# LioQing/wgpu-3dgs-core

Hardware: AMD Instinct MI355X
Metric: Msplats/s @1080p (Gaussians per second through proj+sort+blend; 3 frames in flight on 3 priority streams) (higher is better)
Workload: dtype f32; 1 GPU; 1M synthetic Gaussians, SH degree 0 (ShNone/RotScale 48 B), 1920x1080; gaussians=1000000, visible=708615, pairs=2550276, launches_per_frame=14, parallelism=single GPU, 3 frames in flight on 3 priority streams, frames_in_flight=3, renderer_scratch_copies=3

## Files before the change

### __graft_entry__.py

```python
import os
import sys

ROOT = os.path.dirname(os.path.abspath(__file__))
for p in (ROOT, os.path.join(ROOT, "tools")):
    if p not in sys.path:
        sys.path.insert(0, p)


def build_cpp_mirror_test():
    import subprocess
    out = os.path.join(ROOT, "build")
    os.makedirs(out, exist_ok=True)
    exe = os.path.join(out, "test_mirror")
    subprocess.run(["g++", "-std=c++17", "-O1", "-Wall", "-I" + os.path.join(ROOT, "include"),
                    os.path.join(ROOT, "tests", "cpp", "test_mirror.cpp"), "-o", exe,
                    "-L" + os.path.join(ROOT, "wgpu-3dgs-core_amd", "lib"), "-lgs3d_hip",
                    "-Wl,-rpath,$ORIGIN/../wgpu-3dgs-core_amd/lib"], check=True)
    return exe


def build_cpp_selection_test():
    import subprocess
    out = os.path.join(ROOT, "build")
    os.makedirs(out, exist_ok=True)
    exe = os.path.join(out, "test_selection")
    subprocess.run(["g++", "-std=c++17", "-O1", "-Wall", "-I" + os.path.join(ROOT, "include"),
                    os.path.join(ROOT, "tests", "cpp", "test_selection.cpp"), "-o", exe,
                    "-L" + os.path.join(ROOT, "wgpu-3dgs-core_amd", "lib"), "-lgs3d_hip",
                    "-Wl,-rpath,$ORIGIN/../wgpu-3dgs-core_amd/lib"], check=True)
    return exe


def build_cpp_edit_test():
    import subprocess
    out = os.path.join(ROOT, "build")
    os.makedirs(out, exist_ok=True)
    exe = os.path.join(out, "test_edit")
    subprocess.run(["g++", "-std=c++17", "-O1", "-Wall", "-I" + os.path.join(ROOT, "include"),
                    os.path.join(ROOT, "tests", "cpp", "test_edit.cpp"), "-o", exe,
                    "-L" + os.path.join(ROOT, "wgpu-3dgs-core_amd", "lib"), "-lgs3d_hip",
                    "-Wl,-rpath,$ORIGIN/../wgpu-3dgs-core_amd/lib"], check=True)
    return exe


def build_cpp_history_test():
    import subprocess
    out = os.path.join(ROOT, "build")
    os.makedirs(out, exist_ok=True)
    exe = os.path.join(out, "test_history")
    subprocess.run(["g++", "-std=c++17", "-O1", "-Wall", "-I" + os.path.join(ROOT, "include"),
                    os.path.join(ROOT, "tests", "cpp", "test_history.cpp"), "-o", exe,
                    "-L" + os.path.join(ROOT, "wgpu-3dgs-core_amd", "lib"), "-lgs3d_hip",
                    "-Wl,-rpath,$ORIGIN/../wgpu-3dgs-core_amd/lib"], check=True)
    return exe


def build_cpp_stats_test():
    import subprocess
    out = os.path.join(ROOT, "build")
    os.makedirs(out, exist_ok=True)
    exe = os.path.join(out, "test_stats")
    subprocess.run(["g++", "-std=c++17", "-O1", "-Wall", "-I" + os.path.join(ROOT, "include"),
                    os.path.join(ROOT, "tests", "cpp", "test_stats.cpp"), "-o", exe,
                    "-L" + os.path.join(ROOT, "wgpu-3dgs-core_amd", "lib"), "-lgs3d_hip",
                    "-Wl,-rpath,$ORIGIN/../wgpu-3dgs-core_amd/lib"], check=True)
    return exe


def build_cpp_convert_test():
    import subprocess
    out = os.path.join(ROOT, "build")
    os.makedirs(out, exist_ok=True)
    exe = os.path.join(out, "test_convert")
    subprocess.run(["g++", "-std=c++17", "-O1", "-Wall", "-I" + os.path.join(ROOT, "include"),
                    os.path.join(ROOT, "tests", "cpp", "test_convert.cpp"), "-o", exe,
                    "-L" + os.path.join(ROOT, "wgpu-3dgs-core_amd", "lib"), "-lgs3d_hip",
                    "-Wl,-rpath,$ORIGIN/../wgpu-3dgs-core_amd/lib"], check=True)
    return exe


def build_cpp_contrib_test():
    import subprocess
    out = os.path.join(ROOT, "build")
    os.makedirs(out, exist_ok=True)
    exe = os.path.join(out, "test_contrib")
    subprocess.run(["g++", "-std=c++17", "-O1", "-Wall", "-I" + os.path.join(ROOT, "include"),
                    os.path.join(ROOT, "tests", "cpp", "test_contrib.cpp"), "-o", exe,
                    "-L" + os.path.join(ROOT, "wgpu-3dgs-core_amd", "lib"), "-lgs3d_hip",
                    "-Wl,-rpath,$ORIGIN/../wgpu-3dgs-core_amd/lib"], check=True)
    return exe


def build_cpp_metrics_test():
    import subprocess
    out = os.path.join(ROOT, "build")
    os.makedirs(out, exist_ok=True)
    exe = os.path.join(out, "test_metrics")
    subprocess.run(["g++", "-std=c++17", "-O1", "-Wall", "-I" + os.path.join(ROOT, "include"),
                    os.path.join(ROOT, "tests", "cpp", "test_metrics.cpp"), "-o", exe,
                    "-L" + os.path.join(ROOT, "wgpu-3dgs-core_amd", "lib"), "-lgs3d_hip",
                    "-Wl,-rpath,$ORIGIN/../wgpu-3dgs-core_amd/lib"], check=True)
    return exe


def build_cpp_logf_test():
    import subprocess
    out = os.path.join(ROOT, "build")
    os.makedirs(out, exist_ok=True)
    exe = os.path.join(out, "test_logf")
    subprocess.run(["g++", "-std=c++17", "-O2", "-Wall", "-ffp-contract=off", "-pthread",
                    os.path.join(ROOT, "tests", "cpp", "test_logf.cpp"), "-o", exe], check=True)
    return exe


def build_cpp_fullsize_test():
    import subprocess
    out = os.path.join(ROOT, "build")
    os.makedirs(out, exist_ok=True)
    exe, obj = os.path.join(out, "test_fullsize"), os.path.join(out, "gs_synth.o")
    subprocess.run(["gcc", "-O2", "-std=c11", "-fopenmp", "-c", os.path.join(ROOT, "tools", "gs_synth.c"), "-o", obj], check=True)
    subprocess.run(["g++", "-std=c++17", "-O2", "-Wall", "-I" + os.path.join(ROOT, "include"),
                    os.path.join(ROOT, "tests", "cpp", "test_fullsize.cpp"), obj, "-o", exe, "-fopenmp", "-lm",
                    "-L" + os.path.join(ROOT, "wgpu-3dgs-core_amd", "lib"), "-lgs3d_hip",
                    "-Wl,-rpath,$ORIGIN/../wgpu-3dgs-core_amd/lib"], check=True)
    return exe


def build():
    import importlib.util
    spec = importlib.util.spec_from_file_location(
        "_gs_build", os.path.join(ROOT, "wgpu-3dgs-core_amd", "build.py"))
    b = importlib.util.module_from_spec(spec)
    spec.loader.exec_module(b)
    path = b.build(force=True, verbose=True)
    assert os.path.exists(path)
    from oracle import binding as ob
    ob.build(force=True)
    import synth
    synth.build(force=True)
    build_cpp_mirror_test()
    build_cpp_selection_test()
    build_cpp_edit_test()
    build_cpp_history_test()
    build_cpp_stats_test()
    build_cpp_convert_test()
    build_cpp_contrib_test()
    build_cpp_metrics_test()
    build_cpp_logf_test()
    build_cpp_fullsize_test()
    import wgpu_3dgs_core_amd as gs
    assert gs._capi.load().gs_abi_version() == 1
    print("built:", path)


def smoke():
    import numpy as np
    import synth
    import wgpu_3dgs_core_amd as gs
    from oracle import binding as ob

    dev = gs.Device(0)
    lim = dev.limits()
    print("device:", lim.arch_name.decode(), "CUs", lim.compute_units)
    stream = dev.create_stream()
    pod = gs.GaussianPodWithShSingleCov3dRotScaleConfigs
    g = synth.scene(20000)
    pods = pod.from_gaussian(g)
    W, H = 640, 360
    cam = gs.camera_look_at((0, 0, 0), (0, 0, -1), (0, 1, 0), float(np.deg2rad(60.0)), W, H)
    gt, mt = gs.gaussian_transform_pod(sh_deg=3), gs.model_transform_pod()
    buf = gs.GaussiansBuffer.new_with_pods(dev, pod, pods)
    img = gs.Buffer(dev, size=W * H * 16)
    r = gs.Renderer(dev)
    r.render(stream, buf, gt, mt, cam, img.device_ptr())
    rgba = img.download(stream, np.float32).reshape(H, W, 4)
    st = r.stats()

    ocam = ob.Camera()
    for name, _ in cam._fields_:
        v = getattr(cam, name)
        if hasattr(v, "__len__"):
            getattr(ocam, name)[:] = list(v)
        else:
            setattr(ocam, name, v)
    if os.environ.get("GS3D_RECT_V1") != "1":
        ob.set_rect_version(4 if r.sort_info().tile_masks else 3)
    order = buf.download_order(stream)
    assert np.array_equal(order, ob.spatial_order(pod.sh, pod.cov, pods))
    ref, d, vis, _ = ob.render(pod.sh, pod.cov, pods, ob.gaussian_transform(sh_deg=3),
                               ob.model_transform(), ocam, order=order)
    err = float(np.abs(rgba - ref).max())
    print("smoke: N=%d visible=%d pairs=%d  oracle pairs=%d  RGBA Linf=%g" % (len(g), st.visible, st.pairs, d, err))
    assert st.pairs == d and st.visible == vis
    assert err <= 1e-4, err
    m = gs.image_compare(dev, stream, img.device_ptr(), img.device_ptr(), W, H, ssim=True)
    assert m.identical and m.finite == W * H and m.differing == 0 and m.ssim == 1.0, m
    print("smoke OK")


if __name__ == "__main__":
    build()
    if "--smoke" in sys.argv:
        smoke()
```

### wgpu-3dgs-core_amd/csrc/gs_render_kernels.h

```cpp
#pragma once

#include <type_traits>

#include "gs_device_common.h"

namespace gs {

constexpr int PP_THREADS = 256;
constexpr int PP_ITEMS = 4;
constexpr int PP_CHUNK = PP_THREADS * PP_ITEMS;

struct FrameConsts {
    float M[16];
    float V[16];
    float ISR[9];
    float WS[9];
    float cam_pos[3];
    float fx, fy, cx, cy;
    float near_plane, far_plane;
    float size2, limx, limy, max_std_dev;
    float bg[3];
    uint32_t sh_deg, no_sh0;
    uint32_t width, height;
    uint32_t tiles_x, tiles_y;
    uint32_t band_ty0, band_ty1;
    uint32_t mask_culled_records;
    uint32_t nt_loads;
    uint32_t clip_rect;
    float cull_gain;
    float ellipse_pmin;
    uint32_t rect32;
    uint32_t tile_masks;
    uint32_t wt_stores;
    uint32_t wt_pairs;
    uint32_t wt_records;
};

__host__ __device__ inline uint32_t rect_small_code(uint32_t r0, uint32_t r1, uint32_t rows) {
    const uint32_t w = (r1 & 0xffffu) - (r0 & 0xffffu), h = (r1 >> 16) - (r0 >> 16);
    return (rows & 0xfffu) | ((w - 1u) << 12) | ((h - 1u) << 14);
}
__host__ __device__ inline uint32_t rect_pack32(uint32_t r0, uint32_t r1, uint32_t rows, uint32_t tiles_x) {
    const uint32_t x0 = r0 & 0xffffu, y0 = r0 >> 16, x1 = r1 & 0xffffu, y1 = r1 >> 16;
    const uint32_t origin = y0 * tiles_x + x0;
    if (rows & 0x8000u) return 0x80000000u | (origin << 16) | rect_small_code(r0, r1, rows);
    return (origin << 16) | (x1 - x0 - 1u) | ((y1 - y0 - 1u) << 8);
}
__host__ __device__ inline uint2 rect_pack64(uint32_t r0, uint32_t r1, uint32_t rows) {
    uint2 r;
    r.x = r0;
    r.y = (rows & 0x8000u) ? rect_small_code(r0, r1, rows) << 16 : r1;
    return r;
}
__host__ __device__ inline uint32_t rect_rows_count(uint32_t code) {
    return ((code >> 2) & 3u) + ((code >> 6) & 3u) + ((code >> 10) & 3u);
}
__host__ __device__ inline uint32_t rect_count32(uint32_t p) {
    return (p >> 31) ? rect_rows_count(p) : ((p & 0xffu) + 1u) * (((p >> 8) & 0xffu) + 1u);
}
__host__ __device__ inline uint32_t rect_count64(uint2 r) {
    return (r.y & 0xffffu) == 0u ? rect_rows_count(r.y >> 16)
                                 : ((r.y & 0xffffu) - (r.x & 0xffffu)) * ((r.y >> 16) - (r.x >> 16));
}
__host__ __device__ inline void rect_unpack32(uint32_t p, uint32_t tiles_x, uint32_t &r0, uint32_t &r1, uint32_t &rows) {
    const uint32_t origin = (p >> 16) & 0x7fffu, x0 = origin % tiles_x, y0 = origin / tiles_x;
    const uint32_t w = (p >> 31) ? ((p >> 12) & 3u) + 1u : (p & 0xffu) + 1u, h = (p >> 31) ? ((p >> 14) & 3u) + 1u : ((p >> 8) & 0xffu) + 1u;
    r0 = x0 | (y0 << 16);
    r1 = (x0 + w) | ((y0 + h) << 16);
    rows = (p >> 31) ? 0x8000u | (p & 0xfffu) : 0u;
}
__host__ __device__ inline void rect_unpack64(uint2 r, uint32_t &r0, uint32_t &r1, uint32_t &rows) {
    r0 = r.x;
    if ((r.y & 0xffffu) == 0u && r.y != 0u) {
        const uint32_t c = r.y >> 16, w = ((c >> 12) & 3u) + 1u, h = ((c >> 14) & 3u) + 1u;
        r1 = ((r.x & 0xffffu) + w) | (((r.x >> 16) + h) << 16);
        rows = 0x8000u | (c & 0xfffu);
    } else {
        r1 = r.y;
        rows = 0u;
    }
}

__device__ __forceinline__ void store16(void *p, uint4 v, uint32_t mode) {
    typedef uint32_t u32x4_t __attribute__((ext_vector_type(4)));
    typedef uint32_t u32x4_a4_t __attribute__((ext_vector_type(4), aligned(4)));
    const u32x4_t w = {v.x, v.y, v.z, v.w};
    if (mode == 1u) asm volatile("global_store_dwordx4 %0, %1, off sc1\n\ts_nop 1" ::"v"(p), "v"(w) : "memory");
    else if (mode == 2u) asm volatile("global_store_dwordx4 %0, %1, off nt\n\ts_nop 1" ::"v"(p), "v"(w) : "memory");
    else if (mode == 3u) asm volatile("global_store_dwordx4 %0, %1, off sc0 sc1\n\ts_nop 1" ::"v"(p), "v"(w) : "memory");
    else *(u32x4_a4_t *)p = u32x4_a4_t{v.x, v.y, v.z, v.w};
}


struct FrameState {
    uint32_t visible;
    uint32_t pairs;
    uint32_t overflow;
    uint32_t list_blocks;
    uint32_t list_slots;
    uint32_t cull_ticket;
    uint32_t rank_fault;
    uint32_t rank_inject;
    uint32_t pairs_round1;
    uint32_t round2_visible;
    uint32_t tiles_done;
    uint32_t tiles_open;
    uint32_t round2_skip;
    uint32_t round2_dense;
    uint32_t round1_visible;
    uint32_t depth_tau;
    uint32_t depth_bucket_max;
    uint32_t tile_bucket_max;
};
constexpr uint32_t FRAME_FLAG_PAIR_OVERFLOW = 1u;
constexpr uint32_t FRAME_FLAG_SKIPPED = 2u;
constexpr uint32_t FRAME_FLAG_RANK_FAULT = 4u;

struct FrameResult {
    uint32_t visible;
    uint32_t flags;
    uint64_t pairs_total;
    uint32_t gen;
    uint32_t depth_bucket_max;
    uint32_t tile_bucket_max;
    uint32_t tiles_done;
    uint32_t tiles_open;
    uint32_t round_pairs_max;
    uint32_t pairs_round1;
    uint32_t pad;
};

__device__ __forceinline__ void publish_result(FrameResult *r, uint32_t visible, uint64_t pairs_total, uint32_t flags,
                                               uint32_t gen, uint32_t *flags_dev = nullptr, uint32_t depth_bucket_max = 0u,
                                               uint32_t tile_bucket_max = 0u, uint32_t tiles_done = 0u, uint32_t tiles_open = 0u,
                                               uint32_t round_pairs_max = 0u, uint32_t pairs_round1 = 0u) {
    if (flags_dev) *flags_dev = flags;
    r->visible = visible;
    r->pairs_total = pairs_total;
    r->flags = flags;
    r->depth_bucket_max = depth_bucket_max;
    r->tile_bucket_max = tile_bucket_max;
    r->tiles_done = tiles_done;
    r->tiles_open = tiles_open;
    r->round_pairs_max = round_pairs_max;
    r->pairs_round1 = pairs_round1;
    __hip_atomic_store(&r->gen, gen, __ATOMIC_RELEASE, __HIP_MEMORY_SCOPE_SYSTEM);
}

__global__ void k_publish_result(FrameResult *r, FrameState *state, uint32_t gen, uint32_t *flags_dev) {
    if (threadIdx.x == 0 && blockIdx.x == 0) {
        state->visible = 0;
        state->pairs = 0;
        state->overflow = 0;
        publish_result(r, 0u, 0ull, 0u, gen, flags_dev);
    }
}

// ... 3032 lines not shown
    else if constexpr (OFF == 2) return (uint32_t)__builtin_amdgcn_update_dpp(0, (int)v, 0x4E, 0xf, 0xf, true);
    else if constexpr (OFF == 4) return (uint32_t)__builtin_amdgcn_update_dpp(0, (int)v, 0x141, 0xf, 0xf, true);
    else if constexpr (OFF == 8) return (uint32_t)__builtin_amdgcn_update_dpp(0, (int)v, 0x140, 0xf, 0xf, true);
    else return (uint32_t)__builtin_amdgcn_ds_swizzle((int)v, 0x401F);
}
template <int GL>
__device__ __forceinline__ void contrib_add(unsigned long long *s_qh, uint32_t *s_max, uint32_t acc, float w0, float w1, uint32_t lg) {
    uint32_t q = (uint32_t)(w0 * 16777216.0f) + (uint32_t)(w1 * 16777216.0f);
    uint32_t h = (w0 > 0.0f ? 1u : 0u) + (w1 > 0.0f ? 1u : 0u);
    uint32_t m = f2u(w0) > f2u(w1) ? f2u(w0) : f2u(w1);
#define GS_CONTRIB_FOLD(OFF)                                  \
    if constexpr (GL > OFF) {                                 \
        const uint32_t oq = contrib_other_half<OFF>(q);       \
        const uint32_t oh = contrib_other_half<OFF>(h);       \
        const uint32_t om = contrib_other_half<OFF>(m);       \
        q += oq;                                              \
        h += oh;                                              \
        m = om > m ? om : m;                                  \
    }
    GS_CONTRIB_FOLD(1)
    GS_CONTRIB_FOLD(2)
    GS_CONTRIB_FOLD(4)
    GS_CONTRIB_FOLD(8)
    GS_CONTRIB_FOLD(16)
#undef GS_CONTRIB_FOLD
    if (lg == 0u && h != 0u) {
        (void)__hip_atomic_fetch_add((unsigned long long *)((char *)s_qh + 2u * acc), ((unsigned long long)h << 32) | q, __ATOMIC_RELAXED,
                                     __HIP_MEMORY_SCOPE_WORKGROUP);
        (void)__hip_atomic_fetch_max((uint32_t *)((char *)s_max + acc), m, __ATOMIC_RELAXED, __HIP_MEMORY_SCOPE_WORKGROUP);
    }
}
__device__ __forceinline__ void contrib_flush(const ContribIO &c, uint32_t index, unsigned long long qh, uint32_t m) {
    if ((uint32_t)(qh >> 32) != 0u) {
        uint4 *p = c.rec + index;
        (void)__hip_atomic_fetch_add((unsigned long long *)p, qh & 0xffffffffull, __ATOMIC_RELAXED, __HIP_MEMORY_SCOPE_AGENT);
        (void)__hip_atomic_fetch_add((uint32_t *)p + 2, (uint32_t)(qh >> 32), __ATOMIC_RELAXED, __HIP_MEMORY_SCOPE_AGENT);
        (void)__hip_atomic_fetch_max((uint32_t *)p + 3, m, __ATOMIC_RELAXED, __HIP_MEMORY_SCOPE_AGENT);
    }
}

template <int MODE, int G, bool ROUNDS = false, bool AUX = false, typename... AuxArg>
__global__ __launch_bounds__(BLEND_THREADS) void k_blend_grouped(uint32_t *__restrict__ ranges,
                                                                 const uint32_t *__restrict__ idx,
                                                                 const uint32_t *__restrict__ recs,
                                                                 FrameConsts fc, float4 *__restrict__ rgba,
                                                                 const FrameState *__restrict__ state, TileKeys tk,
                                                                 AuxArg... aux_arg) {
    constexpr bool CONTRIB = is_contrib_pack<AuxArg...>::value;
    static_assert(sizeof...(AuxArg) == (AUX || CONTRIB ? 1u : 0u), "the AUX blend takes one AuxIO, the CONTRIB one one ContribIO, the plain one none");
    static_assert(!CONTRIB || (!AUX && !ROUNDS), "contribution frames take one round and no planes");
    static_assert(G == 2 || G == 4 || G == 8, "lane groups per wave");
    if (state->overflow) return;
    constexpr int GL = WAVE / G;
    constexpr int BW = G == 8 ? 4 : 8;
    constexpr int BH = 2 * GL / BW;
    constexpr int NCOL = 16 / BW;
    constexpr int NROW = 16 / BH;
    constexpr int NL = 2 * G;
    static_assert(NCOL * NROW == NL && G == NCOL * (NROW / 2), "one list per block, G blocks per wave");
    constexpr uint32_t NULL_REC = BLEND_BATCH;
    constexpr uint32_t RS = 48;
    __shared__ __attribute__((aligned(16))) float s_rec[(BLEND_BATCH + 1) * (RS / 4)];
    __shared__ __attribute__((aligned(16))) uint16_t s_list_mem[NL * BLEND_BATCH + (G == 8 ? 2 : 0)];
    uint16_t(*const s_list)[BLEND_BATCH] = (uint16_t(*)[BLEND_BATCH])s_list_mem;
    typedef typename std::conditional<G == 8, uint16_t, uint32_t>::type cnt_t;
    __shared__ __attribute__((aligned(16))) cnt_t s_cnt[2][NL];
    __shared__ uint32_t s_alive[2];

    const uint32_t tid = threadIdx.x, lane = tid & 63u, wid = tid >> 6;
    const uint32_t tile = fc.band_ty0 * fc.tiles_x + blockIdx.x;
    const uint32_t ty = tile / fc.tiles_x, tx = tile % fc.tiles_x;
    const uint32_t gi = lane / GL, lg = lane % GL;
    const uint32_t bx = gi % (uint32_t)NCOL, by = gi / (uint32_t)NCOL;
    const uint32_t px = tx * 16u + bx * (uint32_t)BW + lg % (uint32_t)BW;
    const uint32_t py0 = ty * 16u + wid * 8u + by * BH + lg / (uint32_t)BW, py1 = py0 + BH / 2;
    const float pxf = (float)px + 0.5f;
    const uint32_t my_list = wid * G + gi;
    const float tx0 = (float)(tx * 16u) + 0.5f, ty0 = (float)(ty * 16u) + 0.5f;

    if (ROUNDS && tk.round == 2u && ((tk.done[tile >> 5] >> (tile & 31u)) & 1u)) return;
    uint32_t start, end;
    __shared__ uint32_t s_range[2];
    blend_tile_range_wg(tk, ranges, tile, lane, wid, s_range, start, end);
    f32x2 T = {1.0f, 1.0f}, C0 = {0.0f, 0.0f}, C1 = {0.0f, 0.0f}, C2 = {0.0f, 0.0f};
    const bool in0 = px < fc.width && py0 < fc.height, in1 = px < fc.width && py1 < fc.height;
    constexpr float DEAD = 1.0e15f;
    bool live0 = in0, live1 = in1;
    if (ROUNDS && tk.round == 2u) {
        if (in0) {
            const float4 s = rgba[(uint64_t)py0 * fc.width + px];
            C0.x = s.x; C1.x = s.y; C2.x = s.z; T.x = fabsf(s.w);
            live0 = s.w > 0.0f;
        }
        if (in1) {
            const float4 s = rgba[(uint64_t)py1 * fc.width + px];
            C0.y = s.x; C1.y = s.y; C2.y = s.z; T.y = fabsf(s.w);
            live1 = s.w > 0.0f;
        }
    }
    f32x2 D = {0.0f, 0.0f};
    uint32_t pk0 = PICK_NONE, pk1 = PICK_NONE;
    const AuxIO aux = aux_io(aux_arg...);
    const ContribIO cio = contrib_io(aux_arg...);
    unsigned long long *s_qh = nullptr;
    uint32_t *s_max = nullptr;
    uint32_t my_index = 0u;
    bool flush_pending = false;
    if constexpr (CONTRIB) {
        __shared__ __attribute__((aligned(8))) unsigned long long s_contrib_qh[BLEND_BATCH];
        __shared__ uint32_t s_contrib_max[BLEND_BATCH];
        s_qh = s_contrib_qh;
        s_max = s_contrib_max;
    }
    if (AUX && ROUNDS && tk.round == 2u) {
        if (in0) {
            if (aux.depth) D.x = aux.depth[(uint64_t)py0 * fc.width + px];
            if (aux.pick) pk0 = aux.pick[(uint64_t)py0 * fc.width + px];
        }
        if (in1) {
            if (aux.depth) D.y = aux.depth[(uint64_t)py1 * fc.width + px];
            if (aux.pick) pk1 = aux.pick[(uint64_t)py1 * fc.width + px];
        }
    }
    f32x2 pyf = {live0 ? (float)py0 + 0.5f : DEAD, live1 ? (float)py1 + 0.5f : DEAD};
    uint32_t remaining = __builtin_amdgcn_readfirstlane(
        (uint32_t)__popcll(__ballot(live0)) + (uint32_t)__popcll(__ballot(live1)));
    if (tid == 0) {
        *(float4 *)(s_rec + NULL_REC * (RS / 4)) = make_float4(0.0f, 0.0f, 0.0f, 0.0f);
        *(float4 *)(s_rec + NULL_REC * (RS / 4) + 4) = make_float4(0.0f, 1.0f, 0.0f, 0.0f);
        if constexpr (AUX || CONTRIB) *(float4 *)(s_rec + NULL_REC * (RS / 4) + 8) = make_float4(0.0f, 0.0f, 0.0f, 0.0f);
        else *(float2 *)(s_rec + NULL_REC * (RS / 4) + 8) = make_float2(0.0f, 0.0f);
    }

    for (uint32_t b0 = start; b0 < end; b0 += BLEND_BATCH) {
        if (lane == 0) s_alive[wid] = remaining;
        __syncthreads();
        if constexpr (CONTRIB) {
            if (flush_pending) contrib_flush(cio, my_index, s_qh[tid], s_max[tid]);
            flush_pending = false;
        }
        if ((s_alive[0] | s_alive[1]) == 0u) break;

        if constexpr (G == 8) {
            uint4 *l128 = (uint4 *)&s_list[0][0];
            constexpr uint32_t fill = (NULL_REC * RS) * 0x00010001u;
#pragma unroll
            for (uint32_t q = 0; q < NL * BLEND_BATCH / 8; q += BLEND_THREADS) l128[q + tid] = make_uint4(fill, fill, fill, fill);
        } else {
            uint32_t *l32 = (uint32_t *)&s_list[0][0];
            constexpr uint32_t fill = (NULL_REC * RS) * 0x00010001u;
            for (uint32_t q = tid; q < NL * BLEND_BATCH / 2; q += BLEND_THREADS) l32[q] = fill;
        }
        const uint32_t j = b0 + tid;
        float mx = 0.0f, my = 0.0f, ca = 0.0f, cb = 0.0f, cc = 0.0f, thr = 0.0f;
        const bool have = j < end;
        const bool staging = __builtin_amdgcn_ballot_w64(have) != 0ull;
        if constexpr (CONTRIB) {
            s_qh[tid] = 0ull;
            s_max[tid] = 0u;
        }
        uint64_t m[NL];
        if (!staging) {
#pragma unroll
            for (int l = 0; l < NL; l++) m[l] = 0ull;
        } else {
            if (have) {
                const uint32_t slot = idx[j];
                const uint32_t *rec = recs + (uint64_t)slot * REC_WORDS;
                const u32x4_a4 r0 = *(const u32x4_a4 *)(rec);
                const u32x4_a4 r1 = *(const u32x4_a4 *)(rec + 4);
                const uint32_t r2x = rec[8];
                mx = u2f(r0.x); my = u2f(r0.y); ca = u2f(r0.z); cb = u2f(r0.w); cc = u2f(r1.x);
                float pmin;
                if constexpr (MODE == 0) pmin = fmaxf(-__logf(255.0f * u2f(r1.y)) - 1.0e-3f, -5.6f);
                else pmin = fc.ellipse_pmin;
                thr = (MODE == 0 ? pmin : pmin - 1.0e-3f * fabsf(pmin)) - cull_rounding_slack(mx, my, ca, cb, cc, tx0, ty0);
                *(float4 *)(s_rec + tid * (RS / 4)) = make_float4(mx, my, ca, cb);
                *(float4 *)(s_rec + tid * (RS / 4) + 4) = make_float4(cc, pmin, u2f(r1.y), u2f(r1.z));
                if constexpr (AUX)
                    *(float4 *)(s_rec + tid * (RS / 4) + 8) =
                        make_float4(u2f(r1.w), u2f(r2x), u2f(aux.depth_keys[slot] + aux.key_bias), u2f(slot));
                else if constexpr (CONTRIB) {
                    *(float4 *)(s_rec + tid * (RS / 4) + 8) = make_float4(u2f(r1.w), u2f(r2x), 0.0f, u2f(tid * 4u));
                    my_index = contrib_caller_index(cio, slot);
                }
                else
                    *(float2 *)(s_rec + tid * (RS / 4) + 8) = make_float2(u2f(r1.w), u2f(r2x));
            }
            float bx0 = tx0, by0 = ty0;
            if constexpr (G == 8) asm volatile("" : "+v"(bx0), "+v"(by0));
            if constexpr (MODE == 2) {
#pragma unroll
                for (int l = 0; l < NL; l++) {
                    const int lw = l / G, lgi = l % G;
                    const float rx0 = bx0 + (float)BW * (float)(lgi % NCOL);
                    const float ry0 = by0 + 8.0f * (float)lw + (float)BH * (float)(lgi / NCOL);
                    const float ex = mx - clampf(mx, rx0, rx0 + (float)(BW - 1)), ey = my - clampf(my, ry0, ry0 + (float)(BH - 1));
                    m[l] = __builtin_amdgcn_ballot_w64(have && ex * ex + ey * ey <= 2.26f);
                }
            } else {
                const float rcc = __builtin_amdgcn_rcpf(cc), rca = __builtin_amdgcn_rcpf(ca);
                float c_lo[NCOL], c_hi[NCOL], c_q1[NCOL], c_q0[NCOL], c_t[NCOL];
                uint64_t c_inb[NCOL];
                const uint64_t have_b = __builtin_amdgcn_ballot_w64(have);
#pragma unroll
                for (int c = 0; c < NCOL; c++) {
                    const float x0c = bx0 + (float)BW * (float)c;
                    c_lo[c] = mx - (x0c + (float)(BW - 1));
                    c_hi[c] = mx - x0c;
                    c_inb[c] = __builtin_amdgcn_ballot_w64(c_lo[c] <= 0.0f) & __builtin_amdgcn_ballot_w64(c_hi[c] >= 0.0f);
                    const float dn = fabsf(c_lo[c]) < fabsf(c_hi[c]) ? c_lo[c] : c_hi[c];
                    c_q1[c] = cb * dn;
                    c_q0[c] = ca * dn * dn;
                    c_t[c] = -0.5f * c_q1[c] * rcc;
                }
#pragma unroll
                for (int r = 0; r < NROW; r++) {
                    const float y0r = by0 + (float)(BH * r);
                    const float r_lo = my - (y0r + (float)(BH - 1)), r_hi = my - y0r;
                    const uint64_t r_inb = __builtin_amdgcn_ballot_w64(r_lo <= 0.0f) & __builtin_amdgcn_ballot_w64(r_hi >= 0.0f);
                    const float dn = fabsf(r_lo) < fabsf(r_hi) ? r_lo : r_hi;
                    const float r_q1 = cb * dn, r_q0 = cc * dn * dn;
                    const float r_t = -0.5f * r_q1 * rca;
#pragma unroll
                    for (int c = 0; c < NCOL; c++) {
                        const float tv = __builtin_amdgcn_fmed3f(c_t[c], r_lo, r_hi);
                        const float mv = __builtin_fmaf(__builtin_fmaf(cc, tv, c_q1[c]), tv, c_q0[c]);
                        const float th = __builtin_amdgcn_fmed3f(r_t, c_lo[c], c_hi[c]);
                        const float mh = __builtin_fmaf(__builtin_fmaf(ca, th, r_q1), th, r_q0);
                        const uint64_t keep = (c_inb[c] & r_inb) | __builtin_amdgcn_ballot_w64(!(fmaxf(mv, mh) < thr));
                        const int l = (r / (NROW / 2)) * G + (r % (NROW / 2)) * NCOL + c;
                        m[l] = keep & have_b;
                    }
                    if constexpr (G == 8) __builtin_amdgcn_sched_barrier(0);
                }
            }
        }
        if (lane == 0) {
            if constexpr (G == 8) {
                uint32_t *c32 = (uint32_t *)&s_cnt[wid][0];
#pragma unroll
                for (int l = 0; l < NL; l += 2) c32[l / 2] = (uint32_t)__popcll(m[l]) | ((uint32_t)__popcll(m[l + 1]) << 16);
            } else {
#pragma unroll
                for (int l = 0; l < NL; l++) s_cnt[wid][l] = (uint32_t)__popcll(m[l]);
            }
        }
        __syncthreads();
        if (!staging) {
        } else if constexpr (G == 8) {
            const uint4 *c128 = (const uint4 *)&s_cnt[0][0];
            const uint4 ca4 = c128[0], cb4 = c128[1];
            const uint32_t wv[8] = {ca4.x, ca4.y, ca4.z, ca4.w, cb4.x, cb4.y, cb4.z, cb4.w};
            uint32_t w[8];
#pragma unroll
            for (int q = 0; q < 8; q++) w[q] = (uint32_t)__builtin_amdgcn_readfirstlane(wv[q]);
            const uint32_t swid = (uint32_t)__builtin_amdgcn_readfirstlane(wid);
            const uint32_t dump = (uint32_t)(NL * BLEND_BATCH * sizeof(uint16_t));
#pragma unroll
            for (int l = 0; l < NL; l++) {
                const uint32_t base = swid ? (w[l / 2] >> (16 * (l & 1))) & 0xffffu : 0u;
                const uint32_t pos = __builtin_amdgcn_mbcnt_hi((uint32_t)(m[l] >> 32), __builtin_amdgcn_mbcnt_lo((uint32_t)m[l], 0u));
                const uint32_t at = (pos << 1) + 2u * ((uint32_t)(l * BLEND_BATCH) + base);
                uint32_t to;
                asm("v_cndmask_b32 %0, %1, %2, %3" : "=v"(to) : "v"(dump), "v"(at), "s"(m[l]));
                *(uint16_t *)((char *)s_list_mem + to) = (uint16_t)(tid * RS);
            }
        } else {
            uint32_t lbase[NL];
#pragma unroll
            for (int l = 0; l < NL; l++) lbase[l] = s_cnt[0][l];
            __builtin_amdgcn_sched_barrier(0);
#pragma unroll
            for (int l = 0; l < NL; l++)
                if ((m[l] >> lane) & 1ull) s_list[l][(wid ? lbase[l] : 0u) + mbcnt(m[l])] = (uint16_t)(tid * RS);
        }
        uint32_t trip = 0;
        if constexpr (G == 8) {
            const uint4 c0 = *(const uint4 *)&s_cnt[0][wid * G], c1 = *(const uint4 *)&s_cnt[1][wid * G];
            const uint32_t sum[4] = {c0.x + c1.x, c0.y + c1.y, c0.z + c1.z, c0.w + c1.w};
#pragma unroll
            for (int q = 0; q < 4; q++) {
                const uint32_t lo = sum[q] & 0xffffu, hi = sum[q] >> 16;
                trip = lo > trip ? lo : trip;
                trip = hi > trip ? hi : trip;
            }
        } else {
#pragma unroll
            for (int g = 0; g < G; g++) {
                const uint32_t c = s_cnt[0][wid * G + g] + s_cnt[1][wid * G + g];
                trip = c > trip ? c : trip;
            }
        }
        trip = __builtin_amdgcn_readfirstlane(trip);
        __syncthreads();

        if (remaining != 0u) {
            const uint32_t *mine = (const uint32_t *)s_list[my_list];
            const char *rbase = (const char *)s_rec;
            const uint32_t trips = (trip + 1u) >> 1;
            uint32_t pair = mine[0];
            uint32_t id_A = pair & 0xffffu;
            float4 a_A = *(const float4 *)(rbase + id_A), b_A = *(const float4 *)(rbase + id_A + 16);
#define GS_BLEND_STEP(AREC, BREC, ID)                                                                          \
    {                                                                                                         \
        const float dx = AREC.x - pxf;                                                                        \
        const f32x2 dy = f32x2{AREC.y, AREC.y} - pyf;                                                         \
        const float u = AREC.z * dx, wq = AREC.w * dx;                                                        \
        const f32x2 v = f32x2{BREC.x, BREC.x} * dy;                                                           \
        f32x2 t = f32x2{wq, wq} * dy;                                                                         \
        t = pk_fma(v, dy, t);                                                                                 \
        const f32x2 power = pk_fma(f32x2{u, u}, f32x2{dx, dx}, t);                                            \
        bool p0, p1;                                                                                          \
        if constexpr (MODE == 2) {                                                                            \
            const f32x2 d2 = f32x2{dx * dx, dx * dx} + dy * dy;                                               \
            p0 = d2.x <= 2.25f && BREC.y <= 0.0f;                       \
            p1 = d2.y <= 2.25f && BREC.y <= 0.0f;                                                             \
        } else {                                                                                              \
             \
             \
             \
             \
             \
            p0 = power.x <= 0.0f && power.x >= BREC.y;                                                        \
            p1 = power.y <= 0.0f && power.y >= BREC.y;                                                        \
        }                                                                                                     \
        if (__builtin_amdgcn_ballot_w64(p0 || p1) != 0ull) {                                                  \
            float2 cq;                                                                              \
            float zq = 0.0f;                                   \
            uint32_t sq = 0u;                                                                                 \
            if constexpr (AUX || CONTRIB) {                                                                   \
                const float4 c4 = *(const float4 *)(rbase + ID + 32);                                         \
                cq = make_float2(c4.x, c4.y);                                                                 \
                zq = c4.z;                                                                                    \
                sq = f2u(c4.w);                                                                               \
            } else {                                                                                          \
                cq = *(const float2 *)(rbase + ID + 32);                                                      \
            }                                                                                                 \
            f32x2 alpha;                                                                                      \
            if constexpr (MODE == 0) {                                                                        \
                                                              \
                const f32x2 tt = power * f32x2{1.44269504088896340736f, 1.44269504088896340736f};             \
                const f32x2 tm = tt + f32x2{12582912.0f, 12582912.0f};                                        \
                const f32x2 n = tm - f32x2{12582912.0f, 12582912.0f};                                         \
                const f32x2 f = tt - n;                                                                       \
                f32x2 p = {0x1.5f0896p-10f, 0x1.5f0896p-10f};                                                 \
                p = pk_fma(p, f, f32x2{0x1.3cbf6cp-7f, 0x1.3cbf6cp-7f});                                      \
                p = pk_fma(p, f, f32x2{0x1.c6af6cp-5f, 0x1.c6af6cp-5f});                                      \
                p = pk_fma(p, f, f32x2{0x1.ebfa4ap-3f, 0x1.ebfa4ap-3f});                                      \
                p = pk_fma(p, f, f32x2{0x1.62e430p-1f, 0x1.62e430p-1f});                                      \
                p = pk_fma(p, f, f32x2{1.0f, 1.0f});                                                          \
                const f32x2 e = {u2f(f2u(p.x) + (f2u(tm.x) << 23)), u2f(f2u(p.y) + (f2u(tm.y) << 23))};       \
                const f32x2 oe = f32x2{BREC.z, BREC.z} * e;                                                   \
                alpha = f32x2{fminf(0.99f, oe.x), fminf(0.99f, oe.y)};                                        \
            } else {                                                                                          \
                const float flat = fminf(0.99f, BREC.z);                                                      \
                alpha = f32x2{flat, flat};                                                                    \
            }                                                                                                 \
            const bool act0 = p0 && alpha.x >= (1.0f / 255.0f);                                               \
            const bool act1 = p1 && alpha.y >= (1.0f / 255.0f);                                               \
                              \
                                    \
            f32x2 alpha_eff = {act0 ? alpha.x : 0.0f, act1 ? alpha.y : 0.0f};                                 \
            f32x2 test_T = T * (f32x2{1.0f, 1.0f} - alpha_eff);                                               \
                 \
                                                                 \
            const bool fin0 = test_T.x < 0.0001f, fin1 = test_T.y < 0.0001f;                                  \
            const uint64_t f0 = __builtin_amdgcn_ballot_w64(fin0), f1 = __builtin_amdgcn_ballot_w64(fin1);    \
            if ((f0 | f1) != 0ull) {                  \
                if (fin0) { pyf.x = DEAD; alpha_eff.x = 0.0f; test_T.x = T.x; }                               \
                if (fin1) { pyf.y = DEAD; alpha_eff.y = 0.0f; test_T.y = T.y; }                               \
                remaining -= (uint32_t)__popcll(f0) + (uint32_t)__popcll(f1);                                 \
            }                                                                                                 \
            const f32x2 wgt = alpha_eff * T;                                                                  \
            C0 = pk_fma(f32x2{BREC.w, BREC.w}, wgt, C0);                                                      \
            C1 = pk_fma(f32x2{cq.x, cq.x}, wgt, C1);                                                          \
            C2 = pk_fma(f32x2{cq.y, cq.y}, wgt, C2);                                                          \
            if constexpr (AUX) {                                                                              \
                D = pk_fma(f32x2{zq, zq}, wgt, D);                                                            \
                pk0 = alpha_eff.x > 0.0f && T.x > aux.tcut ? sq : pk0;                                        \
                pk1 = alpha_eff.y > 0.0f && T.y > aux.tcut ? sq : pk1;                                        \
            }                                                                                                 \
            if constexpr (CONTRIB) {   \
                if (__builtin_amdgcn_ballot_w64(wgt.x > 0.0f || wgt.y > 0.0f) != 0ull)                        \
                    contrib_add<GL>(s_qh, s_max, sq, wgt.x, wgt.y, lg);                                       \
// ... 126 lines not shown
```

Before: 4617 Msplats/s.

## Replace per-sub-block quadratic minimum test with per-row ellipse x-interval culling

Replaces the per-(row,column) sub-block ellipse test, which evaluated two clamped quadratic minima per cell, with a per-row computation of the ellipse's horizontal extent (one pair of square roots per row). Each column then needs only two comparisons against that interval. Inactive lanes get dummy coefficients so the interval comes out empty. The aim is fewer ALU ops and ballots in the blend kernel's staging cull, at the cost of sqrt ops and new numeric slack terms that could change which blocks are kept.

```diff
diff --git a/__graft_entry__.py b/__graft_entry__.py
--- a/__graft_entry__.py
+++ b/__graft_entry__.py
@@ -110,6 +110,16 @@
     exe = os.path.join(out, "test_logf")
     subprocess.run(["g++", "-std=c++17", "-O2", "-Wall", "-ffp-contract=off", "-pthread",
                     os.path.join(ROOT, "tests", "cpp", "test_logf.cpp"), "-o", exe], check=True)
+    return exe
+
+
+def build_cpp_block_cull_test():
+    import subprocess
+    out = os.path.join(ROOT, "build")
+    os.makedirs(out, exist_ok=True)
+    exe = os.path.join(out, "test_block_cull")
+    subprocess.run(["g++", "-std=c++17", "-O2", "-Wall", "-ffp-contract=off", "-pthread",
+                    os.path.join(ROOT, "tests", "cpp", "test_block_cull.cpp"), "-o", exe], check=True)
     return exe
 
 
@@ -147,6 +157,7 @@
     build_cpp_contrib_test()
     build_cpp_metrics_test()
     build_cpp_logf_test()
+    build_cpp_block_cull_test()
     build_cpp_fullsize_test()
     import wgpu_3dgs_core_amd as gs
     assert gs._capi.load().gs_abi_version() == 1
diff --git a/wgpu-3dgs-core_amd/csrc/gs_block_cull.h b/wgpu-3dgs-core_amd/csrc/gs_block_cull.h
--- /dev/null
+++ b/wgpu-3dgs-core_amd/csrc/gs_block_cull.h
@@ -0,0 +1,102 @@
+#pragma once
+#include <stdint.h>
+
+#if defined(__HIPCC__) || defined(__CUDACC__)
+#define GS_CULL_HD __host__ __device__ __forceinline__
+#else
+#define GS_CULL_HD inline
+#endif
+
+namespace gs_cull {
+
+GS_CULL_HD float rcp1(float x) {
+#if defined(__HIP_DEVICE_COMPILE__)
+    return __builtin_amdgcn_rcpf(x);
+#else
+    return 1.0f / x;
+#endif
+}
+GS_CULL_HD float sqrt1(float x) {
+#if defined(__HIP_DEVICE_COMPILE__)
+    return __builtin_amdgcn_sqrtf(x);
+#else
+    return __builtin_sqrtf(x);
+#endif
+}
+GS_CULL_HD float med3(float a, float lo, float hi) {
+#if defined(__HIP_DEVICE_COMPILE__)
+    return __builtin_amdgcn_fmed3f(a, lo, hi);
+#else
+    if (a != a) return lo < hi ? lo : hi;
+    return a < lo ? lo : (a > hi ? hi : a);
+#endif
+}
+
+GS_CULL_HD float tile_reach(float mx, float my, float x0, float y0) {
+    const float ax = __builtin_fmaxf(__builtin_fabsf(mx - x0), __builtin_fabsf(mx - (x0 + 15.0f)));
+    const float ay = __builtin_fmaxf(__builtin_fabsf(my - y0), __builtin_fabsf(my - (y0 + 15.0f)));
+    return __builtin_fmaxf(ax, ay);
+}
+
+GS_CULL_HD float interval_slack(float ca, float cb, float cc, float d) {
+    return (4.0e-7f * ((__builtin_fabsf(ca) + __builtin_fabsf(cb)) + __builtin_fabsf(cc))) * (d * d);
+}
+
+struct Splat {
+    float km;
+    float dl;
+    float t_hi;
+    float h, g;
+    float tol;
+    bool all;
+};
+
+GS_CULL_HD Splat setup(float ca, float cb, float cc, float thr, float d) {
+    Splat s;
+    const float a4 = 4.0f * ca;
+    const float p = a4 * cc;
+    const float q = cb * cb;
+    const float f = __builtin_fmaf(cb, cb, -q);
+    s.dl = __builtin_fmaf(a4, cc, -q) - f;
+    s.km = (ca * 0x1.000006p+2f) * thr;
+    const float psi2 = (s.km * rcp1(p)) * rcp1(s.dl);
+    s.all = !(s.dl > 0x1p-16f * p) || !(psi2 < 0x1p+120f);
+    const float psi = sqrt1(psi2);
+    s.t_hi = cb * psi;
+    s.h = rcp1(-2.0f * ca);
+    s.g = cb * s.h;
+    s.tol = __builtin_fmaf(__builtin_fabsf(s.g) * 0x1.8p-22f, d, (psi * cc) * -0x1p-20f);
+    return s;
+}
+
+GS_CULL_HD void row(const Splat &s, float r_lo, float r_hi, float &xl, float &xr) {
+    const float tu = med3(s.t_hi, r_lo, r_hi), tl = med3(-s.t_hi, r_lo, r_hi);
+    const float du = __builtin_fmaf(-(s.dl * tu), tu, s.km), dw = __builtin_fmaf(-(s.dl * tl), tl, s.km);
+    xr = __builtin_fmaf(s.h, sqrt1(du), __builtin_fmaf(s.g, tu, s.tol));
+    xl = __builtin_fmaf(-s.h, sqrt1(dw), __builtin_fmaf(s.g, tl, -s.tol));
+}
+
+template <int NCOL, int NROW>
+GS_CULL_HD uint32_t tile_verdicts(float mx, float my, float ca, float cb, float cc, float pmin_eff, float x0, float y0) {
+    constexpr int BW = 16 / NCOL, BH = 16 / NROW;
+    const float d = tile_reach(mx, my, x0, y0);
+    const float thr = pmin_eff - interval_slack(ca, cb, cc, d);
+    const Splat s = setup(ca, cb, cc, thr, d);
+    float c_lo[NCOL], c_hi[NCOL];
+    for (int c = 0; c < NCOL; c++) {
+        const float x0c = x0 + (float)(BW * c);
+        c_lo[c] = mx - (x0c + (float)(BW - 1));
+        c_hi[c] = mx - x0c;
+    }
+    uint32_t out = 0u;
+    for (int r = 0; r < NROW; r++) {
+        const float y0r = y0 + (float)(BH * r);
+        float xl, xr;
+        row(s, my - (y0r + (float)(BH - 1)), my - y0r, xl, xr);
+        for (int c = 0; c < NCOL; c++)
+            if (s.all || (xr >= c_lo[c] && xl <= c_hi[c])) out |= 1u << (c + NCOL * r);
+    }
+    return out;
+}
+
+}
diff --git a/wgpu-3dgs-core_amd/csrc/gs_render_kernels.h b/wgpu-3dgs-core_amd/csrc/gs_render_kernels.h
--- a/wgpu-3dgs-core_amd/csrc/gs_render_kernels.h
+++ b/wgpu-3dgs-core_amd/csrc/gs_render_kernels.h
@@ -3,6 +3,7 @@
 #include <type_traits>
 
 #include "gs_device_common.h"
+#include "gs_block_cull.h"
 
 namespace gs {
 
@@ -3341,7 +3342,8 @@
             for (uint32_t q = tid; q < NL * BLEND_BATCH / 2; q += BLEND_THREADS) l32[q] = fill;
         }
         const uint32_t j = b0 + tid;
-        float mx = 0.0f, my = 0.0f, ca = 0.0f, cb = 0.0f, cc = 0.0f, thr = 0.0f;
+        float mx = 0.0f, my = 0.0f, ca = MODE == 2 ? 0.0f : -1.0f, cb = 0.0f, cc = MODE == 2 ? 0.0f : -1.0f, thr = MODE == 2 ? 0.0f : 1.0f;
+        float reach = 0.0f;
         const bool have = j < end;
         const bool staging = __builtin_amdgcn_ballot_w64(have) != 0ull;
         if constexpr (CONTRIB) {
@@ -3363,7 +3365,8 @@
                 float pmin;
                 if constexpr (MODE == 0) pmin = fmaxf(-__logf(255.0f * u2f(r1.y)) - 1.0e-3f, -5.6f);
                 else pmin = fc.ellipse_pmin;
-                thr = (MODE == 0 ? pmin : pmin - 1.0e-3f * fabsf(pmin)) - cull_rounding_slack(mx, my, ca, cb, cc, tx0, ty0);
+                reach = gs_cull::tile_reach(mx, my, tx0, ty0);
+                thr = (MODE == 0 ? pmin : pmin - 1.0e-3f * fabsf(pmin)) - gs_cull::interval_slack(ca, cb, cc, reach);
                 *(float4 *)(s_rec + tid * (RS / 4)) = make_float4(mx, my, ca, cb);
                 *(float4 *)(s_rec + tid * (RS / 4) + 4) = make_float4(cc, pmin, u2f(r1.y), u2f(r1.z));
                 if constexpr (AUX)
@@ -3377,7 +3380,7 @@
                     *(float2 *)(s_rec + tid * (RS / 4) + 8) = make_float2(u2f(r1.w), u2f(r2x));
             }
             float bx0 = tx0, by0 = ty0;
-            if constexpr (G == 8) asm volatile("" : "+v"(bx0), "+v"(by0));
+            if constexpr (G == 8 || MODE != 2) asm volatile("" : "+v"(bx0), "+v"(by0));
             if constexpr (MODE == 2) {
 #pragma unroll
                 for (int l = 0; l < NL; l++) {
@@ -3388,38 +3391,24 @@
                     m[l] = __builtin_amdgcn_ballot_w64(have && ex * ex + ey * ey <= 2.26f);
                 }
             } else {
-                const float rcc = __builtin_amdgcn_rcpf(cc), rca = __builtin_amdgcn_rcpf(ca);
-                float c_lo[NCOL], c_hi[NCOL], c_q1[NCOL], c_q0[NCOL], c_t[NCOL];
-                uint64_t c_inb[NCOL];
-                const uint64_t have_b = __builtin_amdgcn_ballot_w64(have);
+                const gs_cull::Splat cs = gs_cull::setup(ca, cb, cc, thr, reach);
+                const uint64_t all_b = __builtin_amdgcn_ballot_w64(cs.all);
+                float c_lo[NCOL], c_hi[NCOL];
 #pragma unroll
                 for (int c = 0; c < NCOL; c++) {
                     const float x0c = bx0 + (float)BW * (float)c;
                     c_lo[c] = mx - (x0c + (float)(BW - 1));
                     c_hi[c] = mx - x0c;
-                    c_inb[c] = __builtin_amdgcn_ballot_w64(c_lo[c] <= 0.0f) & __builtin_amdgcn_ballot_w64(c_hi[c] >= 0.0f);
-                    const float dn = fabsf(c_lo[c]) < fabsf(c_hi[c]) ? c_lo[c] : c_hi[c];
-                    c_q1[c] = cb * dn;
-                    c_q0[c] = ca * dn * dn;
-                    c_t[c] = -0.5f * c_q1[c] * rcc;
                 }
 #pragma unroll
                 for (int r = 0; r < NROW; r++) {
                     const float y0r = by0 + (float)(BH * r);
-                    const float r_lo = my - (y0r + (float)(BH - 1)), r_hi = my - y0r;
-                    const uint64_t r_inb = __builtin_amdgcn_ballot_w64(r_lo <= 0.0f) & __builtin_amdgcn_ballot_w64(r_hi >= 0.0f);
-                    const float dn = fabsf(r_lo) < fabsf(r_hi) ? r_lo : r_hi;
-                    const float r_q1 = cb * dn, r_q0 = cc * dn * dn;
-                    const float r_t = -0.5f * r_q1 * rca;
+                    float xl, xr;
+                    gs_cull::row(cs, my - (y0r + (float)(BH - 1)), my - y0r, xl, xr);
 #pragma unroll
                     for (int c = 0; c < NCOL; c++) {
-                        const float tv = __builtin_amdgcn_fmed3f(c_t[c], r_lo, r_hi);
-                        const float mv = __builtin_fmaf(__builtin_fmaf(cc, tv, c_q1[c]), tv, c_q0[c]);
-                        const float th = __builtin_amdgcn_fmed3f(r_t, c_lo[c], c_hi[c]);
-                        const float mh = __builtin_fmaf(__builtin_fmaf(ca, th, r_q1), th, r_q0);
-                        const uint64_t keep = (c_inb[c] & r_inb) | __builtin_amdgcn_ballot_w64(!(fmaxf(mv, mh) < thr));
                         const int l = (r / (NROW / 2)) * G + (r % (NROW / 2)) * NCOL + c;
-                        m[l] = keep & have_b;
+                        m[l] = (__builtin_amdgcn_ballot_w64(xr >= c_lo[c]) & __builtin_amdgcn_ballot_w64(xl <= c_hi[c])) | all_b;
                     }
                     if constexpr (G == 8) __builtin_amdgcn_sched_barrier(0);
                 }
```

Measured after the change: 4647 Msplats/s, median of 6. About the same (+0.6%).
